# tarepan/DDSP-SVC-official

Hardware: AMD Instinct MI355X
Metric: audio samples/sec @44.1kHz CombSub synth (higher is better)
Workload: dtype f32 storage and accumulation; products of the GEMM / FIR contractions split-bf16x3 (hi*hi+hi*lo+lo*hi), of the attention split-bf16 from three pieces (6 products) for the feature projections and two (3 products) for the context sums; everything else f32; `value_fp32_mfma` is the leg with every produ; 1 GPU; CombSub 44.1 kHz, batch=64x2 s per GPU (Fr=172, T=88064), units/f0/volume/spk_id -> audio, seeded random weights, in-kernel noise

## Files before the change

ddsp-svc-official_amd/csrc/fir_synth.hip:

```cpp
#include "gemm_f32.h"
#include "tables.h"

#include <stdlib.h>

namespace {

__global__ void __launch_bounds__(256) fir_act_kernel(int mode, const float* __restrict__ ctrl, int64_t ld, int M, int Mp,
                                                      int ldo, int64_t rows, float* __restrict__ out, int split) {
    const int lane = threadIdx.x & 63;
    const int64_t row = (int64_t)blockIdx.x * 4 + (threadIdx.x >> 6);
    if (row >= rows) return;
    const float* src = ctrl + row * ld;
    if (mode != DDSP_FIR_ALLPASS) {
        float* dst = out + row * ldo;
        const float scale = (mode == DDSP_FIR_STATIC) ? (1.0f / 128.0f) : 1.0f;
        if (split) {
            for (int f0 = 0; f0 < M; f0 += 64) {
                const int f = f0 + lane;
                const float v = f < M ? expf(src[f]) * scale : 0.f;
                const uint32_t w = ddsp_split1_group8(v, lane);
                if (f < M) ((uint32_t*)dst)[f] = w;
            }
            return;
        }
// ... 63 lines not shown
struct EpiMirrorStore {
    float* ir;
    int n;
    __device__ __forceinline__ float col(int) const { return 0.f; }
    __device__ __forceinline__ void operator()(int, int m, int k, float v, float) const {
        float* row = ir + (int64_t)m * n;
        row[k] = v;
        if (k > 0 && k < n / 2) row[n - k] = v;
    }
};

struct EpiEvenOdd {
    float* ir;
    int n;
    static constexpr bool kDual = true;
    __device__ __forceinline__ float col(int) const { return 0.f; }
    __device__ __forceinline__ void operator()(int, int m, int k, float e, float o) const {
        float* row = ir + (int64_t)m * n;
        row[k] = e + o;
        if (k > 0 && k < n / 2) row[n - k] = e - o;
    }
};

__global__ void __launch_bounds__(256) fir_act_exp8_kernel(float scale, const float* __restrict__ ctrl, int64_t ld, int M, int ldo,
                                                           int64_t rows, float* __restrict__ out, int split) {
    const int per_row = M / 8;
    const int64_t i = (int64_t)blockIdx.x * 256 + threadIdx.x;
    if (i >= rows * per_row) return;
    const int64_t row = i / per_row;
    const int gq = (int)(i % per_row);
    const float* src = ctrl + row * ld + 8 * gq;
    const f32x4 a = *(const f32x4*)src, b = *(const f32x4*)(src + 4);
    float v[8];
#pragma unroll
    for (int e = 0; e < 4; ++e) {
        v[e] = expf(a[e]) * scale;
        v[4 + e] = expf(b[e]) * scale;
    }
    float* dst = out + row * ldo + 8 * gq;
    if (split) {
        ddsp_u32x4 hi, lo;
        ddsp_split8(v, hi, lo);
        *(ddsp_u32x4*)dst = hi;
        *(ddsp_u32x4*)(dst + 4) = lo;
    } else {
        *(f32x4*)dst = f32x4{v[0], v[1], v[2], v[3]};
        *(f32x4*)(dst + 4) = f32x4{v[4], v[5], v[6], v[7]};
    }
}

template <int CTRL, int ROW_MASK>
__device__ __forceinline__ double act_dpp_d(double v) {
    const uint64_t u = __builtin_bit_cast(uint64_t, v);
    const int lo = __builtin_amdgcn_update_dpp(0, (int)(uint32_t)u, CTRL, ROW_MASK, 0xf, false);
    const int hi = __builtin_amdgcn_update_dpp(0, (int)(uint32_t)(u >> 32), CTRL, ROW_MASK, 0xf, false);
    return __builtin_bit_cast(double, ((uint64_t)(uint32_t)hi << 32) | (uint32_t)lo);
}
__global__ void __launch_bounds__(256) fir_act_allpass4_kernel(const float* __restrict__ ctrl, int64_t ld, int M, int Mp, int ldo,
                                                               int64_t rows, float* __restrict__ out, int split) {
    const int lane = threadIdx.x & 63;
    const int64_t row = (int64_t)blockIdx.x * 4 + (threadIdx.x >> 6);
    if (row >= rows) return;
    const float* src = ctrl + row * ld;
    float* dst = out + row * ldo;
    const float pi_f = 3.14159274101257324f;
    double carry = 0.0;
    for (int f0 = 0; f0 < Mp; f0 += 256) {
        const int f = f0 + 4 * lane;
        const bool in = f < M, st = f < Mp;
        f32x4 x = {0.f, 0.f, 0.f, 0.f};
        if (in) x = *(const f32x4*)(src + f);
        double run = 0.0, loc[4];
#pragma unroll
        for (int e = 0; e < 4; ++e) {
            const float gd = in ? __fmul_rn(pi_f, tanhf(x[e])) : 0.f;
            run += (double)gd;
            loc[e] = run;
        }
        double incl = run;
        incl += act_dpp_d<0x111, 0xf>(incl);
        incl += act_dpp_d<0x112, 0xf>(incl);
        incl += act_dpp_d<0x114, 0xf>(incl);
        incl += act_dpp_d<0x118, 0xf>(incl);
        incl += act_dpp_d<0x142, 0xa>(incl);
// ... 5 lines not shown
            const float phi = (float)(base + loc[e]);
            float s_ = 0.f, c_ = 0.f;
            if (in) sincosf(phi, &s_, &c_);
            c[e] = c_;
            sn[e] = s_;
        }
        {
            const uint64_t u = __builtin_bit_cast(uint64_t, incl);
            const uint32_t lo = __builtin_amdgcn_readlane((int)(uint32_t)u, 63), hi = __builtin_amdgcn_readlane((int)(uint32_t)(u >> 32), 63);
            carry += __builtin_bit_cast(double, ((uint64_t)hi << 32) | lo);
        }
        if (split) {
            const ddsp_u32x4 pc = ddsp_split4_pair(c, (lane & 1) != 0, 1), ps = ddsp_split4_pair(sn, (lane & 1) != 0, 1);
            if (st) {
                *(ddsp_u32x4*)(dst + f) = pc;
                *(ddsp_u32x4*)(dst + Mp + f) = ps;
            }
        } else if (st) {
            *(f32x4*)(dst + f) = c;
            *(f32x4*)(dst + Mp + f) = sn;
        }
    }
}

__global__ void __launch_bounds__(256) repack_rows_kernel(const float* __restrict__ src, int n, int64_t rows, int ld,
                                                          float* __restrict__ dst) {
    typedef float f32x2r __attribute__((ext_vector_type(2)));
    const int half = ld / 2;
    const int64_t total = rows * half;
    for (int64_t i = (int64_t)blockIdx.x * blockDim.x + threadIdx.x; i < total; i += (int64_t)gridDim.x * blockDim.x) {
        const int64_t m = i / half;
        const int k = 2 * (int)(i % half);
        f32x2r v = {0.f, 0.f};
        if (k < n) v = *(const f32x2r*)(src + m * n + k);
        *(f32x2r*)(dst + m * ld + k) = v;
    }
}

__global__ void __launch_bounds__(256) dyn_window_scale_kernel(float* __restrict__ d_ir, const float* __restrict__ f0,
                                                               int n, int64_t rows, float sr15) {
    const int64_t total = rows * n;
    for (int64_t i = (int64_t)blockIdx.x * blockDim.x + threadIdx.x; i < total; i += (int64_t)gridDim.x * blockDim.x) {
        const int64_t m = i / n;
        const int k = (int)(i % n);
        const float hw = __fdiv_rn(sr15, __fadd_rn(f0[m], 1e-3f));
        float w = __fdiv_rn((float)(k - n / 2), hw);
// ... 115 lines not shown
        g.B_split = tab_split;
        if (presplit) {
            g.A_split = 1;
            g.B = tab_split;
        }
        if (tap_major)
            gemm::launch<true, true, gemm::A_PLAIN>(st, g, 1, epi);
        else
            gemm::launch<true, false, gemm::A_PLAIN>(st, g, 1, epi);
    };
    const int64_t ldb = tap_major ? K : ddsp_pad4(n);
    if (mode == DDSP_FIR_ALLPASS) {
        gemm::Args g = gemm::make(act, lda, tab, ldb, (int)rows, n / 2 + 1, K);
        run(g, EpiEvenOdd{ir, n});
    } else {
        gemm::Args g = gemm::make(act, lda, tab, ldb, (int)rows, n / 2 + 1, K);
        if (mode == DDSP_FIR_DYNAMIC)
            run(g, EpiDynWindow{ir, n, f0_frames, 1.5f * (float)sr, (tap_major && ctx->math != DDSP_MATH_FP32) ? 1 : 0});
        else
            run(g, EpiMirrorStore{ir, n});
    }
    ddsp_prof_end(ctx, st, mode == DDSP_FIR_ALLPASS ? 2.0 * rows * (double)(n / 2 + 1) * 2 * M : 2.0 * rows * (double)n * K,
                  4.0 * rows * (K + n));
    DDSP_LAUNCH_CHECK(ctx);
    return DDSP_OK;
}

extern "C" int ddsp_fir_from_ctrl_bwd(ddsp_ctx* ctx, void* stream, int mode, const float* ctrl, int64_t ctrl_ld,
                                      int n_mag, const float* f0_frames, int64_t rows, int sr, float* d_ir,
                                      float* d_ctrl, int64_t d_ctrl_ld) {
    DDSP_REQUIRE(ctx, ctx && ctrl && d_ir && d_ctrl, "ddsp_fir_from_ctrl_bwd: null argument");
    DDSP_REQUIRE(ctx, mode >= 0 && mode <= 2, "ddsp_fir_from_ctrl_bwd: unknown mode");
    DDSP_REQUIRE(ctx, n_mag >= 3 && n_mag <= 1024 && ctrl_ld >= n_mag && d_ctrl_ld >= n_mag && rows >= 0 && rows < (1 << 30),
                 "ddsp_fir_from_ctrl_bwd: bad shape");
    DDSP_REQUIRE(ctx, mode != DDSP_FIR_DYNAMIC || f0_frames, "ddsp_fir_from_ctrl_bwd: DYNAMIC needs f0_frames");
    if (rows == 0) return DDSP_OK;
    hipStream_t st = (hipStream_t)stream;
    DDSP_ENTER_DEVICE(ctx);
    const int M = n_mag, n = 2 * (n_mag - 1);
    const int K = (mode == DDSP_FIR_ALLPASS) ? 2 * M : M;
    const int lda = ddsp_pad4(K);
    const int ldp = ddsp_pad4(n);
    const bool repack = ctx->math != DDSP_MATH_FP32 && ldp % 32 == 0 && rows >= 1024;
    int rc = ddsp_scratch_reserve_bytes(ctx, (size_t)rows * (lda + (repack ? ldp : 0)) * sizeof(float) + 8192);
    if (rc) return rc;
    ddsp_scratch_reset(ctx);
// ... 33 lines not shown
```

ddsp-svc-official_amd/csrc/gemm_f32.h:

```cpp
#pragma once
#include "common.h"

#include <stdlib.h>
#include <type_traits>

namespace gemm {

enum { A_PLAIN = 0, A_CONV3 = 1, A_FRAMES = 2, A_CONVK = 3, A_DWCONV = 4 };

struct Args {
    const float* A;
    const float* B;
    int M, N, K;
    int64_t lda, ldb;
    int zdiv;
    int64_t sA_hi, sA_lo, sB_hi, sB_lo;
    int Fr, Cin;
    int tap_shift;
    int ktaps, dil;
    float in_slope;
    const float* zeros;
    int sub_from, parent_tn;
    int math;
    const float* B_split;
// ... 742 lines not shown
    g.K = K;
    g.lda = lda;
    g.ldb = ldb;
    g.zdiv = 1;
    g.sA_hi = g.sA_lo = g.sB_hi = g.sB_lo = 0;
    g.Fr = 1;
    g.Cin = 4;
    g.tap_shift = 0;
    g.ktaps = 3;
    g.dil = 1;
    g.in_slope = 1.f;
    g.zeros = nullptr;
    g.sub_from = 0;
    g.parent_tn = 0;
    g.math = 0;
    g.B_split = nullptr;
    g.A_split = 0;
    g.xcd_cut = 0;
    g.xcd = -1;
    g.kz = 0;
    return g;
}

struct EpiStore {
    float* C;
    int64_t ldc;
    const float* bias;
    int zdiv;
    int64_t sC_hi, sC_lo;
    __device__ __forceinline__ float col(int n) const { return bias ? bias[n] : 0.f; }
    __device__ __forceinline__ void operator()(int z, int m, int n, float v, float cb) const {
        float* c = C + (int64_t)(z / zdiv) * sC_hi + (int64_t)(z % zdiv) * sC_lo;
        c[(int64_t)m * ldc + n] = v + cb;
    }
    static constexpr bool kStore4 = true;
    __device__ __forceinline__ bool vec_ok() const {
        return ((uintptr_t)C % 16) == 0 && ldc % 4 == 0 && sC_hi % 4 == 0 && sC_lo % 4 == 0;
    }
    __device__ __forceinline__ void store4(int z, int m, int n, f32x4 v) const {
        float* c = C + (int64_t)(z / zdiv) * sC_hi + (int64_t)(z % zdiv) * sC_lo;
        if (bias) v += *(const f32x4_u*)(bias + n);
        *(f32x4*)(c + (int64_t)m * ldc + n) = v;
    }
};

struct EpiResidual {
// ... 19 lines not shown
```

ddsp-svc-official_amd/ddsp/vocoder.py:

```python
import os

import torch
import yaml

import hipddsp
from hipddsp import (COMB_SINC, COMB_SINC_GATED, COMB_NONE, EXC_AUDIO, EXC_GENERATE, EXC_UNIT_NOISE, FIR_ALLPASS,
                     FIR_DYNAMIC, FIR_STATIC, FIR_SPLIT_BF16)

from .analysis import (Audio2HubertSoft, F0_Extractor, Units_Encoder, Volume_Extractor,
                       _find_torchcrepe_checkpoint, align_units)
from .unit2control import Unit2Control


class DotDict(dict):

    def __getattr__(self, key):
        val = self.get(key)
        return DotDict(val) if type(val) is dict else val

    __setattr__ = dict.__setitem__
    __delattr__ = dict.__delitem__


def load_model(model_path, device="cpu"):
# ... 33 lines not shown
        self._hop = int(block_size)

    def _context(self, f0_frames, ragged=False):
        if not f0_frames.is_cuda:
            raise RuntimeError("the synthesiser runs on a HIP device only (no CPU fallback): move the model and its "
                               "inputs to 'cuda'")
        if ragged and self._hop % 4:
            raise ValueError("n_frames= needs a block_size that is a multiple of 4")
        return hipddsp.context_for(f0_frames.device)

    def _scan(self, ctx, f0_frames, initial_phase, infer):
        return ctx.phase_scan(f0_frames, self._hop, self._sr, initial_phase, bool(infer), self._comb_mode,
                              **self._front_wants)

    def _render(self, ctx, ctrl, ps, f0_frames, excitation, n_dev=None, keep=False):
        raise NotImplementedError

    def _crop(self, ctx, n_dev, Fr):
        return (lambda *xs: ctx.ragged_crop_(n_dev, Fr, self._hop, *xs)) if n_dev is not None else (lambda *xs: None)

    def _stages(self, ctx, n_dev, Fr, keep):
        saved = [] if keep else None
        return self._crop(ctx, n_dev, Fr), saved, (saved.extend if keep else (lambda xs: None))

    def _ragged_noise(self, ctx, n_dev, B, Fr, noise, noise_seed):
        seed = 0 if noise is not None else (hipddsp.seed_from_torch() if noise_seed is None else int(noise_seed))
        return ctx.ragged_noise(noise, seed, n_dev, B, Fr, self._hop), EXC_UNIT_NOISE, 0

    @staticmethod
    def _noise_args(noise, noise_seed):
        if noise is not None:
            return noise.contiguous().float(), EXC_UNIT_NOISE, 0
        return None, EXC_GENERATE, (hipddsp.seed_from_torch() if noise_seed is None else int(noise_seed))

    def _phase_out(self, ctx, ps, n_dev=None):
        if self._front_wants.get("want_phase"):
            if n_dev is not None:
                ctx.ragged_crop_(n_dev, ps["phase_frames"].shape[1], self._hop, ps["phase"])
            return ps["phase"]
        pf = ps["phase_frames"]
        return pf if n_dev is None else ctx.ragged_frames(pf, n_dev, hold=False, out=pf)

    @staticmethod
    def _result(phase, outs):
        return outs[0], phase.unsqueeze(-1), tuple(outs[1:]) or (outs[0], outs[0])

# ... 116 lines not shown
class CombSub(_SynthBase):

    def __init__(self, sampling_rate, block_size, n_mag_allpass, n_mag_harmonic, n_mag_noise, n_unit=256, n_spk=1,
                 c=False):
        super().__init__(sampling_rate, block_size)
        print(" [DDSP Model] Combtooth Subtractive Synthesiser (Old Version)")
        self.n_mags = (int(n_mag_allpass), int(n_mag_harmonic), int(n_mag_noise))
        self.unit2ctrl = Unit2Control(n_unit, n_spk, {"group_delay": n_mag_allpass,
                                                      "harmonic_magnitude": n_mag_harmonic,
                                                      "noise_magnitude": n_mag_noise}, c)

    _comb_mode = COMB_SINC
    _front_wants = {}
    _n_outs = 3

    def _render(self, ctx, ctrl, ps, f0_frames, excitation, n_dev=None, keep=False):
        B, Fr = ctrl.shape[0], ctrl.shape[1]
        rows, sr, hop = B * Fr, self._sr, self._hop
        na, nh, nn_ = self.n_mags
        c2 = ctrl.reshape(rows, -1)
        crop, saved, save = self._stages(ctx, n_dev, Fr, keep)
        comb = ps["comb"]
        crop(comb)
        ir = ctx.fir_from_ctrl(FIR_ALLPASS, c2, 0, na, rows, sr)
        h, _ = ctx.ltv_fir(comb, ir, B, Fr, hop, math=ctx.fir_math)
        crop(h)
        save((comb, h, ir))
        ir = ctx.fir_from_ctrl(FIR_DYNAMIC, c2, na, nh, rows, sr, f0_frames)
        harmonic, _ = ctx.ltv_fir(h, ir, B, Fr, hop, math=ctx.fir_math)
        crop(harmonic)
        save((ir,))
        ir = ctx.fir_from_ctrl(FIR_STATIC, c2, na + nh, nn_, rows, sr)
        nz, exc, seed = excitation()
        noise_out, signal = ctx.ltv_fir(nz, ir, B, Fr, hop, excitation=exc, noise_seed=seed, add_in=harmonic,
                                        math=ctx.fir_math)
        crop(noise_out, signal)
        save((ir,))
        return (signal, harmonic, noise_out), saved

    def _train_backward(self, ctx, ctrl, saved, f0_frames, nargs, d_outs, crop):
        comb, h1, ir_ap, ir_h, ir_n = saved
        d_signal, d_harm, d_noise = d_outs
        B, Fr = ctrl.shape[0], ctrl.shape[1]
        rows, sr, hop = B * Fr, self._sr, self._hop
        na, nh, nn_ = self.n_mags
        nz, exc, seed = nargs
        d_h = _sum_grads(comb, d_signal, d_harm)
        d_n = _sum_grads(comb, d_signal, d_noise)
        c2 = ctrl.reshape(rows, -1)
        d_ctrl = torch.empty_like(c2)
        _, d_ir = ctx.ltv_fir_bwd(nz, ir_n, d_n, B, Fr, hop, excitation=exc, noise_seed=seed, want_d_audio=False)
        ctx.fir_from_ctrl_bwd(FIR_STATIC, c2, na + nh, nn_, rows, sr, d_ir, d_ctrl)
        d_h1, d_ir = ctx.ltv_fir_bwd(h1, ir_h, d_h, B, Fr, hop)
        crop(d_h1)
        ctx.fir_from_ctrl_bwd(FIR_DYNAMIC, c2, na, nh, rows, sr, d_ir, d_ctrl, f0_frames)
# ... 9 lines not shown

class Sins(_SynthBase):

    def __init__(self, sampling_rate, block_size, n_harmonics, n_mag_allpass, n_mag_noise, n_unit=256, n_spk=1,
                 c=False):
        super().__init__(sampling_rate, block_size)
        print(" [DDSP Model] Sinusoids Additive Synthesiser")
        self.n_mags = (int(n_harmonics), int(n_mag_allpass), int(n_mag_noise))
        self.unit2ctrl = Unit2Control(n_unit, n_spk, {"amplitudes": n_harmonics, "group_delay": n_mag_allpass,
                                                      "noise_magnitude": n_mag_noise}, c)

    _comb_mode = COMB_NONE
    _front_wants = {"want_phase": True}
    _n_outs = 3

    def _render(self, ctx, ctrl, ps, f0_frames, excitation, n_dev=None, keep=False):
        B, Fr = ctrl.shape[0], ctrl.shape[1]
        rows, sr, hop = B * Fr, self._sr, self._hop
        nhm, na, nn_ = self.n_mags
        c2 = ctrl.reshape(rows, -1)
        crop, saved, save = self._stages(ctx, n_dev, Fr, keep)
        sinusoids = ctx.sins_bank(c2, 0, nhm, f0_frames, ps["phase"], B, Fr, hop, sr)
        crop(sinusoids)
        ir = ctx.fir_from_ctrl(FIR_ALLPASS, c2, nhm, na, rows, sr)
        harmonic, _ = ctx.ltv_fir(sinusoids, ir, B, Fr, hop, math=ctx.fir_math)
        crop(harmonic)
        save((ps["phase"], sinusoids, ir))
        ir = ctx.fir_from_ctrl(FIR_STATIC, c2, nhm + na, nn_, rows, sr)
        nz, exc, seed = excitation()
        noise_out, signal = ctx.ltv_fir(nz, ir, B, Fr, hop, excitation=exc, noise_seed=seed, add_in=harmonic,
                                        math=ctx.fir_math)
        crop(noise_out, signal)
        save((ir,))
        return (signal, harmonic, noise_out), saved

    def _train_backward(self, ctx, ctrl, saved, f0_frames, nargs, d_outs, crop):
        phase, sinusoids, ir_ap, ir_n = saved
        d_signal, d_harm, d_noise = d_outs
        B, Fr = ctrl.shape[0], ctrl.shape[1]
        rows, sr, hop = B * Fr, self._sr, self._hop
        nhm, na, nn_ = self.n_mags
        nz, exc, seed = nargs
        d_h = _sum_grads(sinusoids, d_signal, d_harm)
        d_n = _sum_grads(sinusoids, d_signal, d_noise)
        c2 = ctrl.reshape(rows, -1)
        d_ctrl = torch.empty_like(c2)
        _, d_ir = ctx.ltv_fir_bwd(nz, ir_n, d_n, B, Fr, hop, excitation=exc, noise_seed=seed, want_d_audio=False)
        ctx.fir_from_ctrl_bwd(FIR_STATIC, c2, nhm + na, nn_, rows, sr, d_ir, d_ctrl)
        d_sin, d_ir = ctx.ltv_fir_bwd(sinusoids, ir_ap, d_h, B, Fr, hop)
        crop(d_sin)
        ctx.fir_from_ctrl_bwd(FIR_ALLPASS, c2, nhm, na, rows, sr, d_ir, d_ctrl)
# ... 46 lines not shown
```

ddsp-svc-official_amd/hipddsp/__init__.py:

```python
import ctypes
import numbers
import os
import threading

import torch

_HERE = os.path.dirname(os.path.abspath(__file__))
LIB_PATH = os.path.join(_HERE, "libddsp_amd.so")

DDSP_OK, DDSP_ERR_ARG, DDSP_ERR_HIP, DDSP_ERR_OOM = 0, -1, -2, -3

COMB_NONE, COMB_SINC, COMB_SINC_GATED = 0, 1, 2
FIR_ALLPASS, FIR_DYNAMIC, FIR_STATIC = 0, 1, 2
EXC_AUDIO, EXC_UNIT_NOISE, EXC_GENERATE = 0, 1, 2
FIR_FP32, FIR_SPLIT_BF16 = 0, 3
ABI_VERSION = 7
MATH_FP32, MATH_SPLIT_BF16 = 0, 3
ATTENTION_CAUSAL = 200
SLICER_PAD = {"constant": 0, "reflect": 1}
ATTENTION_PAIR = 100

_c = ctypes
_vp, _i64, _u64, _int, _f32, _f64 = _c.c_void_p, _c.c_int64, _c.c_uint64, _c.c_int, _c.c_float, _c.c_double

# ... 63 lines not shown
        for (name, _, _), t in zip(self._slots, tensors):
            if not t.is_cuda:
                raise RuntimeError(f"{self.owner} parameters must live on a HIP device (no CPU fallback)")
            t = t.detach()
            if not t.is_contiguous() or t.dtype != torch.float32:
                if not self.copy:
                    raise ValueError(f"{self.owner} parameters must be contiguous fp32")
                t = t.contiguous().float()
            keep.append(t)
            setattr(w, name, t.data_ptr())
        w.version = 0 if uncached else (self._nonce + 1 + sum(int(t._version) for t in tensors)) & ((1 << 64) - 1)
        if all(a.data_ptr() == b.data_ptr() for a, b in zip(keep, tensors)):
            self._ws = (key, w, keep)
        return w, keep


class DatasetView(_c.Structure):
    _fields_ = ([(n, _vp) for n in ("audio", "units", "f0", "volume", "audio_off", "audio_len", "frame_off", "frames",
                                    "spk_id", "duration", "next_valid")]
                + [("n_files", _i64), ("total_frames", _i64)]
                + [(n, _c.c_int32) for n in ("n_aunit", "n_unit", "hop", "sample_rate", "fp16")])


class ProfEntry(_c.Structure):
    _fields_ = [("family", _int), ("name", _c.c_char * 36), ("launches", _i64), ("ms_total", _c.c_double),
                ("flops_total", _c.c_double), ("bytes_total", _c.c_double)]


CONV_X_SPLIT, CONV_ACT_SPLIT = 1, 2


def presplit(w):
    if w.dtype != torch.float32 or w.shape[-1] % 8:
        raise ValueError("presplit: fp32 with a multiple of 8 columns")
    g = w.contiguous().reshape(*w.shape[:-1], w.shape[-1] // 8, 8)
    hi = g.to(torch.bfloat16)
    lo = (g - hi.float()).to(torch.bfloat16)
    return torch.cat([hi, lo], dim=-1).contiguous().view(torch.float32).reshape(w.shape)


FAMILIES = ["phase_scan", "fir_act", "fir_dft_gemm", "ltv_fir", "u2c_prep", "u2c_gemm_conv3", "u2c_gemm_linear",
            "u2c_gemm_feat", "u2c_gemm_ctx", "u2c_gemm_attnout", "u2c_rowwise", "sins_bank", "spectral_ola", "rss_loss",
            "sola", "upsample", "other", "ltv_fir_bwd", "fir_synth_bwd", "u2c_bwd", "optim"]

SIGNATURES = {
    "ddsp_abi_version": (_int, []),
    "ddsp_ctx_create": (_int, [_c.POINTER(_vp), _int]),
    "ddsp_ctx_destroy": (_int, [_vp]),
    "ddsp_last_error": (_c.c_char_p, [_vp]),
    "ddsp_ctx_reserve": (_int, [_vp, _u64]),
    "ddsp_ctx_poll_error": (_int, [_vp]),
    "ddsp_ctx_set_math": (_int, [_vp, _int]),
    "ddsp_ctx_get_math": (_int, [_vp]),
    "ddsp_upsample": (_int, [_vp, _vp, _vp, _i64, _i64, _i64, _int, _vp]),
    "ddsp_phase_scan": (_int, [_vp, _vp, _vp, _vp, _i64, _i64, _int, _int, _int, _int, _vp, _vp, _vp, _vp, _vp]),
    "ddsp_fir_from_ctrl": (_int, [_vp, _vp, _int, _vp, _i64, _int, _vp, _i64, _int, _vp]),
    "ddsp_ltv_fir_bwd": (_int, [_vp, _vp, _vp, _int, _u64, _vp, _vp, _i64, _i64, _int, _int, _vp, _vp]),
    "ddsp_fir_from_ctrl_bwd": (_int, [_vp, _vp, _int, _vp, _i64, _int, _vp, _i64, _int, _vp, _vp, _i64]),
    "ddsp_sins_bank": (_int, [_vp, _vp, _vp, _i64, _int, _vp, _vp, _i64, _i64, _int, _int, _vp]),
    "ddsp_spectral_ola": (_int, [_vp, _vp, _vp, _i64, _vp, _vp, _int, _u64, _i64, _i64, _int, _vp]),
    "ddsp_sins_bank_bwd": (_int, [_vp, _vp, _vp, _i64, _int, _vp, _vp, _vp, _i64, _i64, _int, _int, _vp, _i64]),
    "ddsp_spectral_ola_bwd": (_int, [_vp, _vp, _vp, _i64, _vp, _vp, _int, _u64, _vp, _i64, _i64, _int, _vp, _i64]),
    "ddsp_rss_loss": (_int, [_vp, _vp, _vp, _vp, _i64, _i64, _c.POINTER(_int), _c.POINTER(_int), _int, _f32, _f32, _vp, _vp]),
    "ddsp_sola": (_int, [_vp, _vp, _vp, _i64, _int, _int, _int, _int, _vp, _vp, _vp]),
    "ddsp_volume_gate": (_int, [_vp, _vp, _vp, _vp, _f32, _i64, _i64, _int]),
    "ddsp_volume_gate_rows": (_int, [_vp, _vp, _vp, _vp, _vp, _vp, _f32, _i64, _i64, _i64, _int]),
    "ddsp_stitch": (_int, [_vp, _vp, _vp, _i64, _vp, _i64]),
    "ddsp_phase_vocoder": (_int, [_vp, _vp, _vp, _vp, _vp, _vp, _int, _vp]),
    "ddsp_volume_extract": (_int, [_vp, _vp, _vp, _i64, _i64, _int, _vp]),
    "ddsp_volume_extract_frac": (_int, [_vp, _vp, _vp, _i64, _i64, _f64, _vp]),
    "ddsp_align_units": (_int, [_vp, _vp, _vp, _i64, _i64, _i64, _i64, _f32, _vp]),
    "ddsp_gemm_res_ln": (_int, [_vp, _vp, _vp, _vp, _vp, _vp, _vp, _vp, _int, _int, _vp, _vp, _int]),
    "ddsp_u2c_dwconv_pw2": (_int, [_vp] * 11 + [_int, _int, _int, _int, _vp, _vp, _vp]),
    "ddsp_conv1d_pair_supported": (_int, [_vp, _int, _int, _int]),
    "ddsp_conv1d_pair": (_int, [_vp, _vp, _vp, _vp, _vp, _vp, _vp, _i64, _int, _int, _int, _f32, _vp, _vp]),
    "ddsp_retime_f0": (_int, [_vp, _vp, _vp, _i64, _f64, _f64, _f32, _f64, _i64, _vp]),
    "ddsp_resample_length": (_i64, [_i64, _int, _int]),
    "ddsp_resample": (_int, [_vp, _vp, _vp, _i64, _i64, _int, _int, _int, _vp]),
    "ddsp_conv1d": (_int, [_vp, _vp, _vp, _vp, _vp, _i64, _int, _int, _int, _int, _f32, _vp, _vp, _vp, _f32, _vp, _int]),
# ... 490 lines not shown
            self.call("ddsp_unit2ctrl_fwd_keep", ctypes.byref(weights), *args, _ptr(keep), nbytes, _ptr(ctrl))
        return ctrl, keep

    def unit2ctrl_bwd_kept(self, weights, grads, units, f0_frames, phase_frames, volume, spk_id, spk_mix_dict, keep, d_ctrl,
                           n_frames=None):
        d_ctrl = d_ctrl.contiguous().float()
        hold, args = self._u2c_inputs(units, f0_frames, phase_frames, volume, spk_id, spk_mix_dict)
        if n_frames is not None:
            self.call("ddsp_unit2ctrl_bwd_kept_ragged", ctypes.byref(weights), *args, _ptr(self._counts_dev(n_frames, units.shape[0])),
                      _ptr(keep), keep.numel(), _ptr(d_ctrl), ctypes.byref(grads))
        else:
            self.call("ddsp_unit2ctrl_bwd_kept", ctypes.byref(weights), *args, _ptr(keep), keep.numel(), _ptr(d_ctrl),
                      ctypes.byref(grads))

    def fir_from_ctrl(self, mode, ctrl2d, col0, n_mag, rows, sr, f0_frames=None):
        ld = ctrl2d.shape[-1]
        n = 2 * (n_mag - 1)
        ir = torch.empty(rows, n, device=ctrl2d.device, dtype=torch.float32)
        base = _ptr(ctrl2d) + 4 * col0
        f0 = None if f0_frames is None else f0_frames.reshape(-1).contiguous().float()
        self.call("ddsp_fir_from_ctrl", int(mode), base, ld, int(n_mag), _ptr(f0), rows, int(sr), _ptr(ir))
        return ir

    def ltv_fir(self, audio, ir, B, Fr, hop, excitation=EXC_AUDIO, noise_seed=0, add_in=None, want_out=True,
                math=FIR_FP32):
        n = ir.shape[-1]
        mk = lambda: torch.empty(B, Fr * hop, device=ir.device, dtype=torch.float32)
        out = mk() if want_out else None
        out_sum = mk() if add_in is not None else None
        self.call("ddsp_ltv_fir", _ptr(audio), int(excitation), int(noise_seed), _ptr(ir), B, Fr, int(hop), int(n),
                  _ptr(add_in), _ptr(out), _ptr(out_sum), int(math))
        return out, out_sum


    def ltv_fir_bwd(self, audio, ir, d_out, B, Fr, hop, excitation=EXC_AUDIO, noise_seed=0, want_d_audio=True,
                    want_d_ir=True):
        n = ir.shape[-1]
        d_out = d_out.contiguous().float()
        d_audio = torch.empty(B, Fr * hop, device=ir.device, dtype=torch.float32) if want_d_audio else None
        d_ir = torch.empty(B * Fr, n, device=ir.device, dtype=torch.float32) if want_d_ir else None
        self.call("ddsp_ltv_fir_bwd", _ptr(audio), int(excitation), int(noise_seed), _ptr(ir), _ptr(d_out), B, Fr,
                  int(hop), int(n), _ptr(d_audio), _ptr(d_ir))
        return d_audio, d_ir

    def fir_from_ctrl_bwd(self, mode, ctrl2d, col0, n_mag, rows, sr, d_ir, d_ctrl2d, f0_frames=None):
        f0 = None if f0_frames is None else f0_frames.reshape(-1).contiguous().float()
# ... 699 lines not shown
```

include/ddsp_amd.h:

```cpp
#ifndef DDSP_AMD_H
#define DDSP_AMD_H

#include <stdint.h>

#ifdef __cplusplus
extern "C" {
#endif

#define DDSP_OK 0
#define DDSP_ERR_ARG (-1)
#define DDSP_ERR_HIP (-2)
#define DDSP_ERR_OOM (-3)

typedef struct ddsp_ctx ddsp_ctx;

int ddsp_ctx_create(ddsp_ctx** out, int device);
int ddsp_ctx_destroy(ddsp_ctx* ctx);
const char* ddsp_last_error(const ddsp_ctx* ctx);
int ddsp_ctx_reserve(ddsp_ctx* ctx, uint64_t bytes);
int ddsp_abi_version(void);
int ddsp_ctx_poll_error(ddsp_ctx* ctx);
#define DDSP_MATH_FP32 0
#define DDSP_MATH_SPLIT_BF16 3
int ddsp_ctx_set_math(ddsp_ctx* ctx, int math);
int ddsp_ctx_get_math(const ddsp_ctx* ctx);

int ddsp_upsample(ddsp_ctx* ctx, void* stream, const float* x, int64_t B, int64_t Fr, int64_t C, int hop,
                  float* out);

#define DDSP_COMB_NONE 0
#define DDSP_COMB_SINC 1
#define DDSP_COMB_SINC_GATED 2
int ddsp_phase_scan(ddsp_ctx* ctx, void* stream, const float* f0_frames, const float* initial_phase, int64_t B,
                    int64_t Fr, int hop, int sr, int precise, int comb_mode, float* rot, float* phase, float* comb,
                    float* f0_up, float* phase_frames);

#define DDSP_FIR_ALLPASS 0
#define DDSP_FIR_DYNAMIC 1
#define DDSP_FIR_STATIC 2
int ddsp_fir_from_ctrl(ddsp_ctx* ctx, void* stream, int mode, const float* ctrl, int64_t ctrl_ld, int n_mag,
                       const float* f0_frames, int64_t rows, int sr, float* ir);

#define DDSP_FIR_FP32 0
#define DDSP_FIR_SPLIT_BF16 3
#define DDSP_EXC_AUDIO 0
#define DDSP_EXC_UNIT_NOISE 1
#define DDSP_EXC_GENERATE 2
int ddsp_ltv_fir(ddsp_ctx* ctx, void* stream, const float* audio, int excitation, uint64_t noise_seed,
                 const float* ir, int64_t B, int64_t Fr, int hop, int n, const float* add_in, float* out,
                 float* out_sum, int math);


typedef struct ddsp_u2c_layer {
    const float *norm_w, *norm_b, *q_w, *q_b, *k_w, *k_b, *v_w, *v_b, *proj, *out_w, *out_b;
    const float *cm_ln_w, *cm_ln_b, *cm_pw1_w, *cm_pw1_b, *cm_dw_w, *cm_dw_b, *cm_pw2_w, *cm_pw2_b;
} ddsp_u2c_layer;

typedef struct ddsp_u2c_weights {
    const float *prenet_conv1_w, *prenet_conv1_b, *prenet_gn_w, *prenet_gn_b, *prenet_conv2_w, *prenet_conv2_b;
    const float *f0_w, *f0_b, *phase_w, *phase_b, *volume_w, *volume_b, *spk_table;
    int n_spk, n_unit, n_out;
    int causal;
    ddsp_u2c_layer layer[3];
    const float *final_ln_w, *final_ln_b, *head_g, *head_v, *head_b;
// ... 331 lines not shown
```

Before: 4.837 billion samples/s.

## Group the per-filter FIR activation and DFT GEMM launches into single grouped kernels

Adds a grouped path that builds all two or three filter impulse responses (allpass, dynamic, static) at once. One kernel computes every activation, and one grouped split-bf16 GEMM kernel with a tile queue across problems and a per-problem epilogue replaces the separate launches. It targets launch overhead and tail underutilisation from several small GEMMs. The path only runs in split-bf16 math with at least 8192 rows and when not keeping saved tensors, and it adds a more complex scheduler.

```diff
diff --git a/ddsp-svc-official_amd/csrc/fir_synth.hip b/ddsp-svc-official_amd/csrc/fir_synth.hip
--- a/ddsp-svc-official_amd/csrc/fir_synth.hip
+++ b/ddsp-svc-official_amd/csrc/fir_synth.hip
@@ -109,10 +109,10 @@
     }
 };
 
-__global__ void __launch_bounds__(256) fir_act_exp8_kernel(float scale, const float* __restrict__ ctrl, int64_t ld, int M, int ldo,
-                                                           int64_t rows, float* __restrict__ out, int split) {
+__device__ __forceinline__ void fir_act_exp8_body(unsigned block, float scale, const float* __restrict__ ctrl, int64_t ld, int M, int ldo,
+                                                  int64_t rows, float* __restrict__ out, int split) {
     const int per_row = M / 8;
-    const int64_t i = (int64_t)blockIdx.x * 256 + threadIdx.x;
+    const int64_t i = (int64_t)block * 256 + threadIdx.x;
     if (i >= rows * per_row) return;
     const int64_t row = i / per_row;
     const int gq = (int)(i % per_row);
@@ -135,6 +135,10 @@
         *(f32x4*)(dst + 4) = f32x4{v[4], v[5], v[6], v[7]};
     }
 }
+__global__ void __launch_bounds__(256) fir_act_exp8_kernel(float scale, const float* __restrict__ ctrl, int64_t ld, int M, int ldo,
+                                                           int64_t rows, float* __restrict__ out, int split) {
+    fir_act_exp8_body(blockIdx.x, scale, ctrl, ld, M, ldo, rows, out, split);
+}
 
 template <int CTRL, int ROW_MASK>
 __device__ __forceinline__ double act_dpp_d(double v) {
@@ -143,10 +147,10 @@
     const int hi = __builtin_amdgcn_update_dpp(0, (int)(uint32_t)(u >> 32), CTRL, ROW_MASK, 0xf, false);
     return __builtin_bit_cast(double, ((uint64_t)(uint32_t)hi << 32) | (uint32_t)lo);
 }
-__global__ void __launch_bounds__(256) fir_act_allpass4_kernel(const float* __restrict__ ctrl, int64_t ld, int M, int Mp, int ldo,
-                                                               int64_t rows, float* __restrict__ out, int split) {
+__device__ __forceinline__ void fir_act_allpass4_body(unsigned block, const float* __restrict__ ctrl, int64_t ld, int M, int Mp, int ldo,
+                                                      int64_t rows, float* __restrict__ out, int split) {
     const int lane = threadIdx.x & 63;
-    const int64_t row = (int64_t)blockIdx.x * 4 + (threadIdx.x >> 6);
+    const int64_t row = (int64_t)block * 4 + (threadIdx.x >> 6);
     if (row >= rows) return;
     const float* src = ctrl + row * ld;
     float* dst = out + row * ldo;
@@ -198,6 +202,43 @@
         }
     }
 }
+__global__ void __launch_bounds__(256) fir_act_allpass4_kernel(const float* __restrict__ ctrl, int64_t ld, int M, int Mp, int ldo,
+                                                               int64_t rows, float* __restrict__ out, int split) {
+    fir_act_allpass4_body(blockIdx.x, ctrl, ld, M, Mp, ldo, rows, out, split);
+}
+
+struct FirActGroup {
+    int n;
+    unsigned first[gemm::GROUP_MAX + 1];
+    int mode[gemm::GROUP_MAX], M[gemm::GROUP_MAX], lda[gemm::GROUP_MAX];
+    const float* ctrl[gemm::GROUP_MAX];
+    float* act[gemm::GROUP_MAX];
+};
+__global__ void __launch_bounds__(256) fir_act_group_kernel(FirActGroup a, int64_t ld, int64_t rows) {
+    int i = 0;
+    while (i + 1 < a.n && blockIdx.x >= a.first[i + 1]) ++i;
+    const unsigned block = blockIdx.x - a.first[i];
+    if (a.mode[i] == DDSP_FIR_ALLPASS)
+        fir_act_allpass4_body(block, a.ctrl[i], ld, a.M[i], (a.M[i] + 31) & ~31, a.lda[i], rows, a.act[i], 1);
+    else
+        fir_act_exp8_body(block, a.mode[i] == DDSP_FIR_STATIC ? 1.0f / 128.0f : 1.0f, a.ctrl[i], ld, a.M[i], a.lda[i], rows, a.act[i], 1);
+}
+
+struct EpiFirGroup {
+    int mode[gemm::GROUP_MAX], n[gemm::GROUP_MAX];
+    float* ir[gemm::GROUP_MAX];
+    const float* f0[gemm::GROUP_MAX];
+    float sr15;
+    __device__ __forceinline__ bool dual(int p) const { return mode[p] == DDSP_FIR_ALLPASS; }
+    template <class F>
+    __device__ __forceinline__ void for_problem(int p, F&& f) const {
+        switch (mode[p]) {
+            case DDSP_FIR_ALLPASS: f(EpiEvenOdd{ir[p], n[p]}); break;
+            case DDSP_FIR_DYNAMIC: f(EpiDynWindow{ir[p], n[p], f0[p], sr15, 1}); break;
+            default: f(EpiMirrorStore{ir[p], n[p]}); break;
+        }
+    }
+};
 
 __global__ void __launch_bounds__(256) repack_rows_kernel(const float* __restrict__ src, int n, int64_t rows, int ld,
                                                           float* __restrict__ dst) {
@@ -359,6 +400,91 @@
     }
     ddsp_prof_end(ctx, st, mode == DDSP_FIR_ALLPASS ? 2.0 * rows * (double)(n / 2 + 1) * 2 * M : 2.0 * rows * (double)n * K,
                   4.0 * rows * (K + n));
+    DDSP_LAUNCH_CHECK(ctx);
+    return DDSP_OK;
+}
+
+extern "C" int ddsp_fir_from_ctrl_group(ddsp_ctx* ctx, void* stream, const float* ctrl, int64_t ctrl_ld, int64_t rows, int sr,
+                                        const ddsp_fir_problem* problems, int n_problems) {
+    DDSP_REQUIRE(ctx, ctx && ctrl && problems, "ddsp_fir_from_ctrl_group: null argument");
+    DDSP_REQUIRE(ctx, n_problems >= 1 && n_problems <= gemm::GROUP_MAX, "ddsp_fir_from_ctrl_group: one to three problems");
+    DDSP_REQUIRE(ctx, rows >= 0 && rows < (1 << 30), "ddsp_fir_from_ctrl_group: bad shape");
+    bool grouped = ctx->math == DDSP_MATH_SPLIT_BF16 && rows >= 8192 && ctrl_ld % 4 == 0;
+    int K[gemm::GROUP_MAX], Ms[gemm::GROUP_MAX], Ns[gemm::GROUP_MAX];
+    for (int i = 0; i < n_problems; ++i) {
+        const ddsp_fir_problem& p = problems[i];
+        DDSP_REQUIRE(ctx, p.ir, "ddsp_fir_from_ctrl_group: null argument");
+        DDSP_REQUIRE(ctx, p.mode >= 0 && p.mode <= 2, "ddsp_fir_from_ctrl_group: unknown mode");
+        DDSP_REQUIRE(ctx, p.n_mag >= 3 && p.n_mag <= 1024 && p.col >= 0 && (int64_t)p.col + p.n_mag <= ctrl_ld,
+                     "ddsp_fir_from_ctrl_group: bad shape");
+        DDSP_REQUIRE(ctx, p.mode != DDSP_FIR_DYNAMIC || p.f0_frames, "ddsp_fir_from_ctrl_group: DYNAMIC needs f0_frames");
+        const int M = p.n_mag;
+        K[i] = p.mode == DDSP_FIR_ALLPASS ? 2 * ddsp_pad32(M) : M;
+        Ms[i] = (int)rows;
+        Ns[i] = M;
+        grouped = grouped && M % 8 == 0 && K[i] % 32 == 0 && (p.mode != DDSP_FIR_ALLPASS || (M % 16 == 0 && K[i] >= 256)) &&
+                  ((uintptr_t)(ctrl + p.col) % 16) == 0;
+    }
+    if (rows == 0) return DDSP_OK;
+    if (!grouped) {
+        for (int i = 0; i < n_problems; ++i) {
+            const ddsp_fir_problem& p = problems[i];
+            const int rc = ddsp_fir_from_ctrl(ctx, stream, p.mode, ctrl + p.col, ctrl_ld, p.n_mag, p.f0_frames, rows, sr, p.ir);
+            if (rc) return rc;
+        }
+        return DDSP_OK;
+    }
+    hipStream_t st = (hipStream_t)stream;
+    DDSP_ENTER_DEVICE(ctx);
+    size_t act_bytes = 4096;
+    for (int i = 0; i < n_problems; ++i) act_bytes += (size_t)rows * K[i] * sizeof(float);
+    int rc = ddsp_scratch_reserve_bytes(ctx, act_bytes);
+    if (rc) return rc;
+    ddsp_scratch_reset(ctx);
+    FirActGroup a = {};
+    float* tab_split[gemm::GROUP_MAX];
+    a.n = n_problems;
+    a.first[0] = 0;
+    double act_traffic = 0.0, flops = 0.0, traffic = 0.0;
+    for (int i = 0; i < n_problems; ++i) {
+        const ddsp_fir_problem& p = problems[i];
+        const int M = p.n_mag, n = 2 * (M - 1);
+        if ((rc = ddsp_scratch_get(ctx, (size_t)rows * K[i] * sizeof(float), (void**)&a.act[i]))) return rc;
+        const int kind = p.mode == DDSP_FIR_ALLPASS ? TAB_IRDFT_CPLX : (p.mode == DDSP_FIR_STATIC ? TAB_IRDFT_RE_HANN : TAB_IRDFT_RE);
+        if ((rc = ddsp_get_table(ctx, st, kind, M, 2, &tab_split[i]))) return rc;
+        a.mode[i] = p.mode;
+        a.M[i] = M;
+        a.lda[i] = K[i];
+        a.ctrl[i] = ctrl + p.col;
+        a.first[i + 1] = a.first[i] + (unsigned)(p.mode == DDSP_FIR_ALLPASS ? ceil_div64(rows, 4) : ceil_div64(rows * (M / 8), 256));
+        act_traffic += 4.0 * rows * (M + K[i]);
+        flops += p.mode == DDSP_FIR_ALLPASS ? 2.0 * rows * (double)(n / 2 + 1) * 2 * M : 2.0 * rows * (double)n * K[i];
+        traffic += 4.0 * rows * (K[i] + n);
+    }
+    ddsp_prof_begin(ctx, st, PF_FIR_ACT);
+    hipLaunchKernelGGL(fir_act_group_kernel, dim3(a.first[n_problems]), dim3(256), 0, st, a, ctrl_ld, rows);
+    ddsp_prof_end(ctx, st, 0.0, act_traffic);
+    DDSP_LAUNCH_CHECK(ctx);
+
+    gemm::GroupArgs ga;
+    EpiFirGroup epi;
+    ga.t = gemm::group_build(n_problems, Ms, Ns, K, 64, 64);
+    epi.sr15 = 1.5f * (float)sr;
+    for (int i = 0; i < gemm::GROUP_MAX; ++i) {
+        const int s = i < ga.t.n ? ga.t.p[i].src : ga.t.p[0].src;
+        const ddsp_fir_problem& p = problems[s];
+        ga.g[i] = gemm::make(a.act[s], K[s], tab_split[s], K[s], (int)rows, Ns[s], K[s]);
+        ga.g[i].math = DDSP_MATH_SPLIT_BF16;
+        ga.g[i].A_split = 1;
+        ga.g[i].B_split = tab_split[s];
+        epi.mode[i] = p.mode;
+        epi.n[i] = 2 * (p.n_mag - 1);
+        epi.ir[i] = p.ir;
+        epi.f0[i] = p.f0_frames;
+    }
+    ddsp_prof_begin(ctx, st, PF_FIR_DFT_GEMM);
+    gemm::launch_dma_group<64, 64>(st, ga, epi);
+    ddsp_prof_end(ctx, st, flops, traffic);
     DDSP_LAUNCH_CHECK(ctx);
     return DDSP_OK;
 }
diff --git a/ddsp-svc-official_amd/csrc/gemm_f32.h b/ddsp-svc-official_amd/csrc/gemm_f32.h
--- a/ddsp-svc-official_amd/csrc/gemm_f32.h
+++ b/ddsp-svc-official_amd/csrc/gemm_f32.h
@@ -1,5 +1,6 @@
 #pragma once
 #include "common.h"
+#include "gemm_group.h"
 
 #include <stdlib.h>
 #include <type_traits>
@@ -788,6 +789,187 @@
     return g;
 }
 
+struct GroupArgs {
+    GroupTable t;
+    Args g[GROUP_MAX];
+};
+
+template <int BM, int BN, class GEpi, int NS = 3, int NW = 4>
+__global__ void __launch_bounds__(64 * NW, (NW == 4 ? 3 : 4)) kernel_dma_group(GroupArgs ga, GEpi epi) {
+    constexpr int WGM = NW / 2, WGN = 2;
+    constexpr int TM = BM / (32 * WGM), TN = BN / (32 * WGN);
+    constexpr int ROWS = BM + BN, STAGE = ROWS * 32, PIECES = ROWS / 8, PPW = PIECES / NW;
+    static_assert(PIECES % NW == 0, "stage must split evenly over the waves");
+    __shared__ __attribute__((aligned(1024))) float lds[NS * STAGE];
+
+    const int tid = threadIdx.x, lane = tid & 63, wave = __builtin_amdgcn_readfirstlane(tid >> 6);
+    const int wm = (wave >> 1) * (BM / WGM), wn = (wave & 1) * (BN / WGN);
+    const int lr = lane & 31, lh = lane >> 5;
+    const int xx = (int)blockIdx.x & 7, xq0 = (int)blockIdx.x >> 3, xgs = (int)gridDim.x >> 3;
+    const int my_tiles = group_my_tiles(ga.t, (int)gridDim.x, (int)blockIdx.x);
+
+    struct Tile {
+        int p, m0, n0, nk;
+    };
+    auto tile_of = [&](int i) -> Tile {
+        int p = 0, mt = 0, nt = 0;
+        group_tile(ga.t, xx, xq0 + i * xgs, &p, &mt, &nt);
+        return Tile{p, mt * BM, nt * BN, ga.t.p[p].nk};
+    };
+    int steps = 0;
+    for (int i = 0; i < my_tiles; ++i) steps += tile_of(i).nk;
+
+    const float* src_cur[PPW];
+    auto tile_src = [&](const Tile& t) {
+        const Args& g = ga.g[t.p];
+#pragma unroll
+        for (int i = 0; i < PPW; ++i) {
+            const int piece = wave + NW * i;
+            const int row = piece * 8 + (lane >> 3);
+            const int slot = (lane & 7) ^ ((row >> 1) & 7);
+            if (row < BM) {
+                int m = t.m0 + row;
+                m = m < g.M ? m : g.M - 1;
+                src_cur[i] = g.A + (int64_t)m * g.lda + slot * 4;
+            } else {
+                int n = t.n0 + row - BM;
+                n = n < g.N ? n : g.N - 1;
+                src_cur[i] = g.B + (int64_t)n * g.ldb + slot * 4;
+            }
+        }
+    };
+    int issued = 0, issue_tile = 0, issue_kt = 0, issue_nk = 0;
+    if (my_tiles > 0) {
+        const Tile t = tile_of(0);
+        issue_nk = t.nk;
+        tile_src(t);
+    }
+    auto issue_next = [&]() {
+        if (issued >= steps) return;
+#pragma unroll
+        for (int i = 0; i < PPW; ++i)
+            __builtin_amdgcn_global_load_lds((const __attribute__((address_space(1))) void*)(src_cur[i] + issue_kt * 32),
+                                             (__attribute__((address_space(3))) void*)(lds + (issued % NS) * STAGE + (wave + NW * i) * 256),
+                                             16, 0, 0);
+        ++issued;
+        if (++issue_kt == issue_nk) {
+            issue_kt = 0;
+            if (++issue_tile < my_tiles) {
+                const Tile t = tile_of(issue_tile);
+                issue_nk = t.nk;
+                tile_src(t);
+            }
+        }
+    };
+#pragma unroll
+    for (int i = 0; i < NS - 1; ++i) issue_next();
+
+    f32x16 acc[TM][TN], acc1[TM][TN];
+#pragma unroll
+    for (int i = 0; i < TM; ++i)
+#pragma unroll
+        for (int j = 0; j < TN; ++j)
+#pragma unroll
+            for (int r = 0; r < 16; ++r) acc[i][j][r] = acc1[i][j][r] = 0.f;
+
+    int kt = 0, tile_i = 0;
+    Tile cur = my_tiles > 0 ? tile_of(0) : Tile{0, 0, 0, 1};
+    for (int step = 0; step < steps; ++step) {
+        static_assert((NS - 2) * PPW <= 63, "vmcnt is a 6-bit counter");
+        if (NS > 2 && step + NS - 2 < steps)
+            asm volatile("s_waitcnt vmcnt(%0)" ::"n"((NS - 2) * PPW) : "memory");
+        else
+            asm volatile("s_waitcnt vmcnt(0)" ::: "memory");
+        __builtin_amdgcn_s_barrier();
+        issue_next();
+        const float* st = lds + (step % NS) * STAGE;
+        f32x4 av[TM][4], bv[TN][4];
+#pragma unroll
+        for (int i = 0; i < TM; ++i) {
+            const int row = wm + 32 * i + lr;
+            const float* rp = st + row * 32;
+#pragma unroll
+            for (int c = 0; c < 4; ++c) av[i][c] = *(const f32x4*)(rp + 4 * ((4 * lh + c) ^ ((row >> 1) & 7)));
+        }
+#pragma unroll
+        for (int j = 0; j < TN; ++j) {
+            const int row = BM + wn + 32 * j + lr;
+            const float* rp = st + row * 32;
+#pragma unroll
+            for (int c = 0; c < 4; ++c) bv[j][c] = *(const f32x4*)(rp + 4 * ((4 * lh + c) ^ ((row >> 1) & 7)));
+        }
+        typedef __bf16 bf16x8 __attribute__((ext_vector_type(8)));
+#pragma unroll
+        for (int half = 0; half < 2; ++half)
+#pragma unroll
+            for (int i = 0; i < TM; ++i)
+#pragma unroll
+                for (int j = 0; j < TN; ++j) {
+                    const bf16x8 ah = __builtin_bit_cast(bf16x8, av[i][2 * half]), al = __builtin_bit_cast(bf16x8, av[i][2 * half + 1]);
+                    const bf16x8 bh = __builtin_bit_cast(bf16x8, bv[j][2 * half]), bl = __builtin_bit_cast(bf16x8, bv[j][2 * half + 1]);
+                    acc[i][j] = __builtin_amdgcn_mfma_f32_32x32x16_bf16(al, bh, acc[i][j], 0, 0, 0);
+                    acc[i][j] = __builtin_amdgcn_mfma_f32_32x32x16_bf16(ah, bl, acc[i][j], 0, 0, 0);
+                    acc[i][j] = __builtin_amdgcn_mfma_f32_32x32x16_bf16(ah, bh, acc[i][j], 0, 0, 0);
+                }
+        ++kt;
+        if (2 * kt == cur.nk && epi.dual(cur.p)) {
+#pragma unroll
+            for (int i = 0; i < TM; ++i)
+#pragma unroll
+                for (int j = 0; j < TN; ++j) {
+                    acc1[i][j] = acc[i][j];
+#pragma unroll
+                    for (int r = 0; r < 16; ++r) acc[i][j][r] = 0.f;
+                }
+        }
+        if (kt == cur.nk) {
+            const Args& g = ga.g[cur.p];
+            const int M = g.M, N = g.N;
+            epi.for_problem(cur.p, [&](const auto& e) {
+                constexpr bool DUAL = epi_is_dual<std::decay_t<decltype(e)>>::value;
+#pragma unroll
+                for (int i = 0; i < TM; ++i)
+#pragma unroll
+                    for (int j = 0; j < TN; ++j) {
+                        const int n = cur.n0 + wn + 32 * j + lr;
+                        const bool n_ok = n < N;
+#pragma unroll
+                        for (int r = 0; r < 16; ++r) {
+                            const int m = cur.m0 + wm + 32 * i + (r & 3) + 8 * (r >> 2) + 4 * lh;
+                            if (n_ok && m < M) {
+                                if constexpr (DUAL)
+                                    e(0, m, n, acc1[i][j][r], acc[i][j][r]);
+                                else
+                                    e(0, m, n, acc[i][j][r], 0.f);
+                            }
+                        }
+                    }
+            });
+#pragma unroll
+            for (int i = 0; i < TM; ++i)
+#pragma unroll
+                for (int j = 0; j < TN; ++j)
+#pragma unroll
+                    for (int r = 0; r < 16; ++r) acc[i][j][r] = 0.f;
+            kt = 0;
+            if (++tile_i < my_tiles) cur = tile_of(tile_i);
+        }
+    }
+}
+
+template <int BM, int BN, int NS, int NW>
+constexpr int group_max_grid() {
+    constexpr int by_lds = 160 * 1024 / (NS * (BM + BN) * 128), by_waves = 16 / NW;
+    return 256 * (by_lds < by_waves ? by_lds : by_waves);
+}
+
+template <int BM, int BN, class GEpi, int NS = 3, int NW = 4>
+inline void launch_dma_group(hipStream_t st, const GroupArgs& ga, const GEpi& epi) {
+    const int grid = group_grid(ga.t, group_max_grid<BM, BN, NS, NW>());
+    if (grid == 0) return;
+    hipLaunchKernelGGL((kernel_dma_group<BM, BN, GEpi, NS, NW>), dim3(grid), dim3(64 * NW), 0, st, ga, epi);
+}
+
 struct EpiStore {
     float* C;
     int64_t ldc;
diff --git a/ddsp-svc-official_amd/csrc/gemm_group.h b/ddsp-svc-official_amd/csrc/gemm_group.h
--- /dev/null
+++ b/ddsp-svc-official_amd/csrc/gemm_group.h
@@ -0,0 +1,93 @@
+#pragma once
+
+#if defined(__HIPCC__)
+#define GEMM_GROUP_HD __host__ __device__ inline
+#else
+#define GEMM_GROUP_HD inline
+#endif
+
+namespace gemm {
+
+constexpr int GROUP_MAX = 3;
+
+struct GroupProblem {
+    int tiles_m, tiles_n;
+    int nk;
+    int src;
+};
+
+struct GroupTable {
+    int n;
+    GroupProblem p[GROUP_MAX];
+};
+
+GEMM_GROUP_HD int group_queue_len(const GroupProblem& p, int x) {
+    const int left = (p.tiles_m % 8) * p.tiles_n;
+    return (p.tiles_m / 8) * p.tiles_n + (left > x ? (left - x + 7) / 8 : 0);
+}
+
+GEMM_GROUP_HD int group_queue_len(const GroupTable& t, int x) {
+    int q = 0;
+    for (int i = 0; i < t.n; ++i) q += group_queue_len(t.p[i], x);
+    return q;
+}
+
+GEMM_GROUP_HD bool group_tile(const GroupTable& t, int x, int q, int* prob, int* mt, int* nt) {
+    for (int i = 0; i < t.n; ++i) {
+        const GroupProblem& p = t.p[i];
+        const int len = group_queue_len(p, x);
+        if (q >= len) {
+            q -= len;
+            continue;
+        }
+        const int own = (p.tiles_m / 8) * p.tiles_n;
+        *prob = i;
+        if (q < own) {
+            *mt = x + 8 * (q / p.tiles_n);
+            *nt = q % p.tiles_n;
+        } else {
+            const int u = (q - own) * 8 + x;
+            *mt = (p.tiles_m / 8) * 8 + u / p.tiles_n;
+            *nt = u % p.tiles_n;
+        }
+        return true;
+    }
+    return false;
+}
+
+GEMM_GROUP_HD int group_my_tiles(const GroupTable& t, int grid, int b) {
+    const int len = group_queue_len(t, b & 7), j = b >> 3, stride = grid >> 3;
+    return j < len ? (len - j + stride - 1) / stride : 0;
+}
+
+inline GroupTable group_build(int n, const int* M, const int* N, const int* K, int BM, int BN) {
+    GroupTable t;
+    t.n = 0;
+    for (int i = 0; i < GROUP_MAX; ++i) t.p[i] = GroupProblem{0, 0, 0, 0};
+    for (int i = 0; i < n && i < GROUP_MAX; ++i) {
+        GroupProblem p{(M[i] + BM - 1) / BM, (N[i] + BN - 1) / BN, K[i] / 32, i};
+        if (p.tiles_m <= 0 || p.tiles_n <= 0 || p.nk <= 0) continue;
+        int at = t.n++;
+        for (; at > 0 && t.p[at - 1].nk < p.nk; --at) t.p[at] = t.p[at - 1];
+        t.p[at] = p;
+    }
+    return t;
+}
+
+inline long group_total_tiles(const GroupTable& t) {
+    long s = 0;
+    for (int i = 0; i < t.n; ++i) s += (long)t.p[i].tiles_m * t.p[i].tiles_n;
+    return s;
+}
+
+inline int group_grid(const GroupTable& t, int max_grid) {
+    int longest = 0;
+    for (int x = 0; x < 8; ++x) {
+        const int len = group_queue_len(t, x);
+        longest = len > longest ? len : longest;
+    }
+    const int grid = 8 * longest;
+    return grid < max_grid ? grid : max_grid;
+}
+
+}
diff --git a/ddsp-svc-official_amd/ddsp/vocoder.py b/ddsp-svc-official_amd/ddsp/vocoder.py
--- a/ddsp-svc-official_amd/ddsp/vocoder.py
+++ b/ddsp-svc-official_amd/ddsp/vocoder.py
@@ -79,6 +79,14 @@
     def _stages(self, ctx, n_dev, Fr, keep):
         saved = [] if keep else None
         return self._crop(ctx, n_dev, Fr), saved, (saved.extend if keep else (lambda xs: None))
+
+    _GROUP_MIN_ROWS = 8192
+
+    def _filters(self, ctx, c2, problems, rows, f0_frames, keep):
+        if keep or rows < self._GROUP_MIN_ROWS:
+            return (ctx.fir_from_ctrl(mode, c2, col, n_mag, rows, self._sr, f0_frames if mode == FIR_DYNAMIC else None)
+                    for mode, col, n_mag in problems)
+        return iter(ctx.fir_from_ctrl_group(c2, problems, rows, self._sr, f0_frames))
 
     def _ragged_noise(self, ctx, n_dev, B, Fr, noise, noise_seed):
         seed = 0 if noise is not None else (hipddsp.seed_from_torch() if noise_seed is None else int(noise_seed))
@@ -241,15 +249,17 @@
         crop, saved, save = self._stages(ctx, n_dev, Fr, keep)
         comb = ps["comb"]
         crop(comb)
-        ir = ctx.fir_from_ctrl(FIR_ALLPASS, c2, 0, na, rows, sr)
+        firs = self._filters(ctx, c2, [(FIR_ALLPASS, 0, na), (FIR_DYNAMIC, na, nh), (FIR_STATIC, na + nh, nn_)], rows,
+                             f0_frames, keep)
+        ir = next(firs)
         h, _ = ctx.ltv_fir(comb, ir, B, Fr, hop, math=ctx.fir_math)
         crop(h)
         save((comb, h, ir))
-        ir = ctx.fir_from_ctrl(FIR_DYNAMIC, c2, na, nh, rows, sr, f0_frames)
+        ir = next(firs)
         harmonic, _ = ctx.ltv_fir(h, ir, B, Fr, hop, math=ctx.fir_math)
         crop(harmonic)
         save((ir,))
-        ir = ctx.fir_from_ctrl(FIR_STATIC, c2, na + nh, nn_, rows, sr)
+        ir = next(firs)
         nz, exc, seed = excitation()
         noise_out, signal = ctx.ltv_fir(nz, ir, B, Fr, hop, excitation=exc, noise_seed=seed, add_in=harmonic,
                                         math=ctx.fir_math)
@@ -305,11 +315,12 @@
         crop, saved, save = self._stages(ctx, n_dev, Fr, keep)
         sinusoids = ctx.sins_bank(c2, 0, nhm, f0_frames, ps["phase"], B, Fr, hop, sr)
         crop(sinusoids)
-        ir = ctx.fir_from_ctrl(FIR_ALLPASS, c2, nhm, na, rows, sr)
+        firs = self._filters(ctx, c2, [(FIR_ALLPASS, nhm, na), (FIR_STATIC, nhm + na, nn_)], rows, f0_frames, keep)
+        ir = next(firs)
         harmonic, _ = ctx.ltv_fir(sinusoids, ir, B, Fr, hop, math=ctx.fir_math)
         crop(harmonic)
         save((ps["phase"], sinusoids, ir))
-        ir = ctx.fir_from_ctrl(FIR_STATIC, c2, nhm + na, nn_, rows, sr)
+        ir = next(firs)
         nz, exc, seed = excitation()
         noise_out, signal = ctx.ltv_fir(nz, ir, B, Fr, hop, excitation=exc, noise_seed=seed, add_in=harmonic,
                                         math=ctx.fir_math)
diff --git a/ddsp-svc-official_amd/hipddsp/__init__.py b/ddsp-svc-official_amd/hipddsp/__init__.py
--- a/ddsp-svc-official_amd/hipddsp/__init__.py
+++ b/ddsp-svc-official_amd/hipddsp/__init__.py
@@ -109,6 +109,10 @@
                 + [(n, _c.c_int32) for n in ("n_aunit", "n_unit", "hop", "sample_rate", "fp16")])
 
 
+class FirProblem(_c.Structure):
+    _fields_ = [("mode", _int), ("col", _int), ("n_mag", _int), ("f0_frames", _vp), ("ir", _vp)]
+
+
 class ProfEntry(_c.Structure):
     _fields_ = [("family", _int), ("name", _c.c_char * 36), ("launches", _i64), ("ms_total", _c.c_double),
                 ("flops_total", _c.c_double), ("bytes_total", _c.c_double)]
@@ -142,6 +146,7 @@
     "ddsp_upsample": (_int, [_vp, _vp, _vp, _i64, _i64, _i64, _int, _vp]),
     "ddsp_phase_scan": (_int, [_vp, _vp, _vp, _vp, _i64, _i64, _int, _int, _int, _int, _vp, _vp, _vp, _vp, _vp]),
     "ddsp_fir_from_ctrl": (_int, [_vp, _vp, _int, _vp, _i64, _int, _vp, _i64, _int, _vp]),
+    "ddsp_fir_from_ctrl_group": (_int, [_vp, _vp, _vp, _i64, _i64, _int, _vp, _int]),
     "ddsp_ltv_fir_bwd": (_int, [_vp, _vp, _vp, _int, _u64, _vp, _vp, _i64, _i64, _int, _int, _vp, _vp]),
     "ddsp_fir_from_ctrl_bwd": (_int, [_vp, _vp, _int, _vp, _i64, _int, _vp, _i64, _int, _vp, _vp, _i64]),
     "ddsp_sins_bank": (_int, [_vp, _vp, _vp, _i64, _int, _vp, _vp, _i64, _i64, _int, _int, _vp]),
@@ -678,6 +683,15 @@
         self.call("ddsp_fir_from_ctrl", int(mode), base, ld, int(n_mag), _ptr(f0), rows, int(sr), _ptr(ir))
         return ir
 
+    def fir_from_ctrl_group(self, ctrl2d, problems, rows, sr, f0_frames=None):
+        f0 = None if f0_frames is None else f0_frames.reshape(-1).contiguous().float()
+        irs = [torch.empty(rows, 2 * (n_mag - 1), device=ctrl2d.device, dtype=torch.float32) for _, _, n_mag in problems]
+        table = (FirProblem * len(problems))(*[
+            FirProblem(int(mode), int(col0), int(n_mag), _ptr(f0) if mode == FIR_DYNAMIC else None, _ptr(ir))
+            for (mode, col0, n_mag), ir in zip(problems, irs)])
+        self.call("ddsp_fir_from_ctrl_group", _ptr(ctrl2d), ctrl2d.shape[-1], rows, int(sr), table, len(problems))
+        return irs
+
     def ltv_fir(self, audio, ir, B, Fr, hop, excitation=EXC_AUDIO, noise_seed=0, add_in=None, want_out=True,
                 math=FIR_FP32):
         n = ir.shape[-1]
diff --git a/include/ddsp_amd.h b/include/ddsp_amd.h
--- a/include/ddsp_amd.h
+++ b/include/ddsp_amd.h
@@ -40,6 +40,16 @@
 #define DDSP_FIR_STATIC 2
 int ddsp_fir_from_ctrl(ddsp_ctx* ctx, void* stream, int mode, const float* ctrl, int64_t ctrl_ld, int n_mag,
                        const float* f0_frames, int64_t rows, int sr, float* ir);
+
+typedef struct ddsp_fir_problem {
+    int mode;
+    int col;
+    int n_mag;
+    const float* f0_frames;
+    float* ir;
+} ddsp_fir_problem;
+int ddsp_fir_from_ctrl_group(ddsp_ctx* ctx, void* stream, const float* ctrl, int64_t ctrl_ld, int64_t rows, int sr,
+                             const ddsp_fir_problem* problems, int n_problems);
 
 #define DDSP_FIR_FP32 0
 #define DDSP_FIR_SPLIT_BF16 3
```

After: 4.925 billion samples/s (median of 6 runs). +1.8%, better.
